# alexlocher/hpmvs

Hardware: AMD Instinct MI355X
Metric: refined_patches_per_sec (higher is better)
Workload: dtype f32 textures / f64 optimiser

## Files before the change

hpmvs_amd/api.py:

```python
from __future__ import annotations

import ctypes as C
import os
from dataclasses import dataclass

import numpy as np

try:
    import torch
except Exception:
    torch = None

HERE = os.path.dirname(os.path.abspath(__file__))
LIB_PATH = os.environ.get("HPMVS_LIB") or os.path.join(HERE, "libhpmvs_amd.so")
MAX_IMAGES = 256
FAST_IMAGES = 64
MAX_LEVELS = 8


class HpmvsError(RuntimeError):
    pass


class Options(C.Structure):
# ... 4 lines not shown

class Camera(C.Structure):
    _fields_ = [("P0", C.c_float * 12), ("center", C.c_float * 4), ("xaxis", C.c_float * 3),
                ("yaxis", C.c_float * 3), ("zaxis", C.c_float * 3), ("fsum", C.c_float), ("n_levels", C.c_int32)]


class PatchBatch(C.Structure):
    _fields_ = [("n", C.c_int32), ("max_images", C.c_int32), ("center", C.c_void_p), ("normal", C.c_void_p),
                ("scale", C.c_void_p), ("n_images", C.c_void_p), ("images", C.c_void_p), ("ok", C.c_void_p),
                ("color", C.c_void_p), ("ncc", C.c_void_p), ("fmin", C.c_void_p), ("x", C.c_void_p),
                ("result", C.c_void_p), ("nevals", C.c_void_p), ("stage", C.c_void_p), ("ngrabs", C.c_void_p)]


class LeafTable(C.Structure):
    _fields_ = [("n", C.c_int32), ("root_center", C.c_float * 3), ("root_width", C.c_float), ("cell_center", C.c_void_p),
                ("cell_width", C.c_void_p), ("patch_center", C.c_void_p), ("born", C.c_void_p), ("died", C.c_void_p)]


class OctreeIndex(C.Structure):
    _fields_ = [("root_center", C.c_float * 3), ("root_width", C.c_float), ("n_branches", C.c_int32), ("n_leaves", C.c_int32),
                ("branch_key", C.c_void_p), ("leaf_key", C.c_void_p)]


class SeedTreeInfo(C.Structure):
    _fields_ = [("root_center", C.c_float * 3), ("root_width", C.c_float), ("scale_floor", C.c_float), ("n_rows", C.c_int32),
                ("n_leaves", C.c_int32)]


EXPORTS = [
    "hpmvs_last_error", "hpmvs_device_count", "hpmvs_build_id", "hpmvs_default_options", "hpmvs_camera_from_nvm",
    "hpmvs_scene_create", "hpmvs_scene_set_view", "hpmvs_scene_set_covis", "hpmvs_scene_commit",
    "hpmvs_scene_destroy", "hpmvs_scene_get_level", "hpmvs_scene_bytes", "hpmvs_build_pyramid",
    "hpmvs_optimize_batch", "hpmvs_init_patches_batch", "hpmvs_objective_batch", "hpmvs_inccs_batch", "hpmvs_last_kernel_ms",
    "hpmvs_last_wide_patches",
    "hpmvs_expand_batch", "hpmvs_expand_directions", "hpmvs_selftest_bobyqa",
    "hpmvs_pack_records", "hpmvs_unpack_records", "hpmvs_allgather_records", "hpmvs_pack_record_tails", "hpmvs_unpack_record_tails",
    "hpmvs_scene_depth_reset", "hpmvs_scene_depth_set_level", "hpmvs_scene_depth_get_level",
    "hpmvs_set_depths_batch", "hpmvs_depth_gates_batch", "hpmvs_depth_footprints_batch", "hpmvs_depth_ops_batch", "hpmvs_level_support_batch",
    "hpmvs_host_alloc", "hpmvs_host_free", "hpmvs_last_staging",
    "hpmvs_undistort", "hpmvs_undistort_map", "hpmvs_scene_set_view_distorted",
    "hpmvs_regularize_batch", "hpmvs_filter_batch", "hpmvs_seed_tree_batch", "hpmvs_octree_locate_batch",
]

_lib = None


def lib():
    global _lib
    if _lib is not None:
        return _lib
    if not os.path.exists(LIB_PATH):
        raise HpmvsError(f"{LIB_PATH} is missing: run `python -c 'import __graft_entry__ as g; g.build()'` "
                         "(there is no fallback implementation)")
    L = C.CDLL(LIB_PATH)
    L.hpmvs_last_error.restype = C.c_char_p
    L.hpmvs_build_id.restype = C.c_char_p
    L.hpmvs_default_options.argtypes = [C.POINTER(Options)]
    L.hpmvs_camera_from_nvm.argtypes = [C.c_double, C.POINTER(C.c_double), C.POINTER(C.c_double), C.c_int, C.c_int,
                                        C.c_int, C.POINTER(Camera)]
    L.hpmvs_scene_create.argtypes = [C.c_int, C.c_int, C.POINTER(C.c_void_p)]
    L.hpmvs_scene_set_view.argtypes = [C.c_void_p, C.c_int, C.c_int, C.c_int, C.c_void_p, C.c_int, C.POINTER(Camera)]
    L.hpmvs_scene_set_covis.argtypes = [C.c_void_p, C.c_int, C.POINTER(C.c_int32), C.c_int]
    L.hpmvs_scene_commit.argtypes = [C.c_void_p]
    L.hpmvs_scene_destroy.argtypes = [C.c_void_p]
    L.hpmvs_scene_get_level.argtypes = [C.c_void_p, C.c_int, C.c_int, C.c_void_p, C.c_size_t, C.POINTER(C.c_int),
                                        C.POINTER(C.c_int)]
    L.hpmvs_scene_bytes.restype = C.c_size_t
# ... 131 lines not shown
        _chk(L.hpmvs_scene_commit(self.h))

    def close(self):
        if self.h:
            lib().hpmvs_scene_destroy(self.h)
            self.h = C.c_void_p()

    def __del__(self):
        try:
            self.close()
        except Exception:
            pass

    def bytes(self) -> int:
        return lib().hpmvs_scene_bytes(self.h)

    def level(self, view: int, level: int) -> np.ndarray:
        w, h = C.c_int(), C.c_int()
        _chk(lib().hpmvs_scene_get_level(self.h, view, level, None, 0, C.byref(w), C.byref(h)))
        out = np.empty((h.value, w.value, 3), dtype=np.uint8)
        _chk(lib().hpmvs_scene_get_level(self.h, view, level, out.ctypes.data, out.nbytes, C.byref(w), C.byref(h)))
        return out

    def last_staging(self):
        a, b = C.c_ulonglong(), C.c_ulonglong()
        _chk(lib().hpmvs_last_staging(self.h, C.byref(a), C.byref(b)))
        return a.value, b.value

    def last_wide_patches(self) -> int:
        n = C.c_int32()
        _chk(lib().hpmvs_last_wide_patches(self.h, C.byref(n)))
        return n.value

    def last_kernel_ms(self) -> float:
        ms = C.c_float()
        _chk(lib().hpmvs_last_kernel_ms(self.h, C.byref(ms)))
        return ms.value


class Batch:

    def __init__(self, center, normal, scale, n_images, images):
        self.n = int(len(scale))
        self.max_images = int(images.shape[1])
        self.center = np.ascontiguousarray(center, dtype=np.float32).copy()
        self.normal = np.ascontiguousarray(normal, dtype=np.float32).copy()
        self.scale = np.ascontiguousarray(scale, dtype=np.float32).copy()
        self.n_images = np.ascontiguousarray(n_images, dtype=np.int32).copy()
        self.images = np.ascontiguousarray(images, dtype=np.int32).copy()
        n = self.n
        self.ok = np.zeros(n, dtype=np.uint8)
        self.color = np.zeros((n, 3), dtype=np.float32)
        self.ncc = np.zeros(n, dtype=np.float32)
        self.fmin = np.zeros(n, dtype=np.float64)
        self.x = np.zeros((n, 3), dtype=np.float64)
        self.result = np.zeros(n, dtype=np.int32)
        self.nevals = np.zeros(n, dtype=np.int32)
        self.stage = np.zeros(n, dtype=np.int32)
        self.ngrabs = np.zeros(n, dtype=np.int32)

    @classmethod
    def from_seeds(cls, seeds, idx=None):
        if idx is None:
            idx = np.arange(len(seeds.scale))
        idx = np.asarray(idx)
        return cls(seeds.center[idx], seeds.normal[idx], seeds.scale[idx], seeds.n_images[idx], seeds.images[idx])
# ... 240 lines not shown
```

hpmvs_amd/csrc/capi.hip:

```cpp
#include <hip/hip_runtime.h>

#include <dlfcn.h>

#include <algorithm>
#include <atomic>
#include <chrono>
#include <cmath>
#include <cstdio>
#include <cstdlib>
#include <cstring>
#include <mutex>
#include <optional>
#include <string>
#include <thread>
#include <time.h>
#include <vector>

#include "../../include/hpmvs_amd.h"
#include "dev_types.h"
#include "launch.h"
#include "octree.hpp"

using namespace hpmvs;

// ... 1726 lines not shown
    HIPCHK(hipGetLastError());
    return c.finish();
}

int hpmvs_depth_footprints_batch(const hpmvs_scene* s, const hpmvs_patch_batch* b, int32_t* writes, int32_t* frees,
                                 int32_t* attached, int32_t* view_block, int on_device, void* stream) {
    int rc = check_depth_batch(s, b, "depth_footprints_batch");
    if (rc) return rc;
    if (!writes && !frees && !attached && !view_block) return fail(HPMVS_ERR_ARG, "depth_footprints_batch: no output array");
    if (b->n == 0) return HPMVS_OK;
    HIPCHK(hipSetDevice(s->device));
    hipStream_t st = (hipStream_t)stream;
    Call c(s, on_device, st);
    const size_t n = (size_t)b->n, M = (size_t)b->max_images, V = (size_t)s->n_views;
    const DevBatch D = c.batch(b, Call::kRead);
    int32_t *dw = c.out(writes, n * M * 4), *df = c.out(frees, n * M * 4);
    int32_t *da = c.out(attached, n * M * 3), *dv = c.out(view_block, n * V * 3);
    if ((rc = c.begin())) return rc;
    launch_depth_footprints(dev_scene(s), s->ddepth, D, dw, df, da, dv, st);
    HIPCHK(hipGetLastError());
    return c.finish();
}

int hpmvs_last_wide_patches(const hpmvs_scene* s, int32_t* n) {
    if (!s || !n) return fail(HPMVS_ERR_ARG, "last_wide_patches: null argument");
    *n = 0;
    if (!s->last_ws) return HPMVS_OK;
    HIPCHK(hipSetDevice(s->device));
    HIPCHK(hipDeviceSynchronize());
    HIPCHK(hipMemcpy(n, s->last_ws + 241, sizeof(int32_t), hipMemcpyDeviceToHost));
    return HPMVS_OK;
}

int hpmvs_debug_counters(const hpmvs_scene* s, unsigned long long* out4) {
    if (!s || !out4) return fail(HPMVS_ERR_ARG, "debug_counters: null argument");
    HIPCHK(hipSetDevice(s->device));
    { const int rcq = service_quiesce(s); if (rcq) return rcq; }
    HIPCHK(hipDeviceSynchronize());
    if (!s->last_queue) return fail(HPMVS_ERR_STATE, "debug_counters: no launch yet");
    HIPCHK(hipMemcpy(out4, (char*)s->last_queue + 16, 544, hipMemcpyDeviceToHost));
    return HPMVS_OK;
}

int hpmvs_last_staging(const hpmvs_scene* s, unsigned long long* staged_bytes, unsigned long long* in_place_bytes) {
    if (!s || !staged_bytes || !in_place_bytes) return fail(HPMVS_ERR_ARG, "last_staging: null argument");
    *staged_bytes = s->last_staged_bytes; *in_place_bytes = s->last_mapped_bytes;
    return HPMVS_OK;
}

void* hpmvs_host_alloc(size_t bytes) {
    void* p = nullptr;
    if (bytes == 0 || hipHostMalloc(&p, bytes, hipHostMallocDefault) != hipSuccess) { (void)hipGetLastError(); return nullptr; }
    return p;
}
void hpmvs_host_free(void* p) {
    if (p && hipHostFree(p) != hipSuccess) (void)hipGetLastError();
}

int hpmvs_last_kernel_ms(const hpmvs_scene* s, float* ms) {
    if (!s || !ms) return fail(HPMVS_ERR_ARG, "last_kernel_ms: null argument");
    if (!s->timed) return fail(HPMVS_ERR_STATE, "last_kernel_ms: no optimize launch yet");
    HIPCHK(hipSetDevice(s->device));
    HIPCHK(hipEventSynchronize(s->ev1));
    HIPCHK(hipEventElapsedTime(ms, s->ev0, s->ev1));
    return HPMVS_OK;
}
// ... 3 lines not shown
```

hpmvs_amd/csrc/kernel_optimize.hip:

```cpp
#include <hip/hip_runtime.h>
#include <atomic>

#include "prof.h"
#define BQ_STATE_LDS 1
#define BQ_STATE_LDS_EXTERN 1
#ifndef BQ_P
#define BQ_P 29
#endif
#define BQ_SLOTS BQ_P
#ifndef HPMVS_STATIC_SLOTS
#define HPMVS_STATIC_SLOTS (!HPMVS_COLD_GLOBAL)
#endif
#ifndef HPMVS_STATIC_MAX_PER_WG
#define HPMVS_STATIC_MAX_PER_WG(W_, kS_) ((W_) * (kS_))
#endif
#ifndef HPMVS_SPREAD_SOLO
#define HPMVS_SPREAD_SOLO 1
#endif
#ifndef HPMVS_COLD_GLOBAL
#define HPMVS_COLD_GLOBAL 0
#endif
#if HPMVS_COLD_GLOBAL
#define BQ_COLD_GLOBAL 1
#ifndef BQ_COLD_LO
#define BQ_COLD_LO 77
#endif
#ifndef BQ_COLD_HI
#define BQ_COLD_HI 138
#endif
#define HPMVS_STATE_ND (164 - (BQ_COLD_HI - BQ_COLD_LO))
#else
#define HPMVS_STATE_ND 164
#endif
#define HPMVS_STATE_NI 13
#define HPMVS_REGION_BYTES (HPMVS_STATE_ND * 8 * BQ_P + HPMVS_STATE_NI * 4 * BQ_P)
#define HPMVS_REGION_KIB ((HPMVS_REGION_BYTES + 1023) / 1024)
#define HPMVS_REGION_16 (HPMVS_REGION_KIB * 64)
#ifndef HPMVS_WG_WAVES
#define HPMVS_WG_WAVES 8
#endif
#ifndef HPMVS_WG_REGIONS
#if HPMVS_COLD_GLOBAL
#define HPMVS_WG_REGIONS 6
#else
#define HPMVS_WG_REGIONS 4
#endif
#endif
#ifdef HPMVS_VARIANT_SUFFIX
#define HPMVS_CAT2(a, b) a##b
#define HPMVS_CAT(a, b) HPMVS_CAT2(a, b)
#define HPMVS_V(name) HPMVS_CAT(name, HPMVS_VARIANT_SUFFIX)
#define HPMVS_VK(name) HPMVS_CAT(name, HPMVS_VARIANT_SUFFIX)
#else
#define HPMVS_VK(name) name
#define HPMVS_V(name) name##_std
#endif
extern __shared__ uint4 hpmvs_dyn[];
#define bq_lds_d ((double*)hpmvs_dyn)
#define bq_lds_i ((int*)((char*)hpmvs_dyn + HPMVS_STATE_ND * 8 * BQ_P))
#include "bobyqa3.hpp"
#include "launch.h"
#include "photometric.hpp"
#include "pipeline.hpp"

namespace hpmvs {

static_assert(BQ_ND_LDS == HPMVS_STATE_ND && BQ_NI == HPMVS_STATE_NI, "state region sized for another layout");

namespace {

constexpr int kP = BQ_P;
constexpr int kRow = 64;
constexpr size_t kCounterBytes = 1024;
constexpr int kPark16 = HPMVS_REGION_16;

#ifndef HPMVS_PARK_AUX
#define HPMVS_PARK_AUX 0
#endif
#ifndef HPMVS_PROXY
#define HPMVS_PROXY 0
#endif
constexpr int kAuxDoubles = 64;
constexpr int kAuxVal = 18;
constexpr int kAuxGrabs = 25;
constexpr int kAuxCtx = 64;
constexpr int kMaxExtra = 7;
typedef __attribute__((address_space(1))) double gdouble;
typedef __attribute__((address_space(1))) float gfloat;
__device__ __forceinline__ void page_in(const uint4* __restrict__ park, uint4* hpmvs_region) {
    const char* g = (const char*)(park + lane_id());
#pragma unroll
    for (int c4 = 0; c4 < HPMVS_REGION_KIB; c4 += 4) {
        asm volatile("" : "+v"(g));
        auto lds = (__attribute__((address_space(3))) void*)(hpmvs_region + c4 * 64);
        auto src = (const __attribute__((address_space(1))) void*)g;
        __builtin_amdgcn_global_load_lds(src, lds, 16, 0, HPMVS_PARK_AUX);
        if (c4 + 1 < HPMVS_REGION_KIB) __builtin_amdgcn_global_load_lds(src, lds, 16, 1024, HPMVS_PARK_AUX);
        if (c4 + 2 < HPMVS_REGION_KIB) __builtin_amdgcn_global_load_lds(src, lds, 16, 2048, HPMVS_PARK_AUX);
        if (c4 + 3 < HPMVS_REGION_KIB) __builtin_amdgcn_global_load_lds(src, lds, 16, 3072, HPMVS_PARK_AUX);
        g += 4096;
    }
    asm volatile("s_waitcnt vmcnt(0)" ::: "memory");
}
#ifndef HPMVS_PARK_NT_STORE
#define HPMVS_PARK_NT_STORE 0
#endif
#if HPMVS_PARK_NT_STORE
#define HPMVS_PARK_ST(dst, v) __builtin_nontemporal_store((v), &(dst))
#else
#define HPMVS_PARK_ST(dst, v) (dst) = (v)
#endif
__device__ __attribute__((noinline)) void page_out(uint4* __restrict__ park, int region_index) {
    typedef unsigned int u4 __attribute__((ext_vector_type(4)));
    typedef __attribute__((address_space(1))) u4 gu4;
    const int lane = lane_id();
    const u4* region = (const u4*)(hpmvs_dyn + region_index * HPMVS_REGION_16);
    gu4* out = (gu4*)(unsigned long long)park;
    int c = 0;
#pragma unroll
    for (; c + 8 <= HPMVS_REGION_KIB; c += 8) {
        const u4 v0 = region[(c + 0) * 64 + lane], v1 = region[(c + 1) * 64 + lane], v2 = region[(c + 2) * 64 + lane],
                    v3 = region[(c + 3) * 64 + lane], v4 = region[(c + 4) * 64 + lane], v5 = region[(c + 5) * 64 + lane],
                    v6 = region[(c + 6) * 64 + lane], v7 = region[(c + 7) * 64 + lane];
        __builtin_amdgcn_sched_barrier(0);
        HPMVS_PARK_ST(out[(c + 0) * 64 + lane], v0); HPMVS_PARK_ST(out[(c + 1) * 64 + lane], v1); HPMVS_PARK_ST(out[(c + 2) * 64 + lane], v2); HPMVS_PARK_ST(out[(c + 3) * 64 + lane], v3);
        HPMVS_PARK_ST(out[(c + 4) * 64 + lane], v4); HPMVS_PARK_ST(out[(c + 5) * 64 + lane], v5); HPMVS_PARK_ST(out[(c + 6) * 64 + lane], v6); HPMVS_PARK_ST(out[(c + 7) * 64 + lane], v7);
        __builtin_amdgcn_sched_barrier(0);
    }
#pragma unroll
    for (; c < HPMVS_REGION_KIB; c++) { const u4 v = region[c * 64 + lane]; HPMVS_PARK_ST(out[c * 64 + lane], v); }
}

}

__device__ __forceinline__ unsigned long long ld_host64(const unsigned long long* p) {
    return __hip_atomic_load(p, __ATOMIC_RELAXED, __HIP_MEMORY_SCOPE_SYSTEM);
}

#ifndef HPMVS_WAVES_PER_EU
#define HPMVS_WAVES_PER_EU 2
#endif
#ifndef HPMVS_BQ_PRIO
#define HPMVS_BQ_PRIO 3
#endif
#ifndef HPMVS_LOCK_SLEEP
#define HPMVS_LOCK_SLEEP 8
#endif
#ifndef HPMVS_A_PRIO
#define HPMVS_A_PRIO 2
#endif
template <bool SERVICE, int W, int R>
__device__ __forceinline__ void optimize_body(DevScene sc, DevOptions o, DevBatch b, int32_t* queue) {
    const int lane = lane_id();
    const int wv = (int)(threadIdx.x >> 6);
    int* const hpmvs_lock = (int*)(hpmvs_dyn + R * HPMVS_REGION_16);
    const int n_wgs = (int)gridDim.x;
    const int gw = wv * n_wgs + (int)blockIdx.x;
    uint16_t* lists = (uint16_t*)((char*)queue + kCounterBytes) + (size_t)gw * kP * kRow;
    uint16_t* row = &lists[(lane < kP ? lane : 0) * kRow];
    uint4* park = (uint4*)((char*)queue + kCounterBytes + (size_t)W * n_wgs * kP * kRow * sizeof(uint16_t)) + (size_t)gw * kPark16;
#if HPMVS_COLD_GLOBAL
    char* cold = (char*)queue + kCounterBytes + (size_t)W * n_wgs * kP * kRow * sizeof(uint16_t) + (size_t)W * n_wgs * kPark16 * 16 +
                 (size_t)W * n_wgs * kP * kRow * sizeof(float) + (size_t)gw * BQ_NCOLD * kP * sizeof(double);
    {
// ... 17 lines not shown
    int px_k = 0;

    constexpr bool service = SERVICE;
    const int per_wg = (b.n + n_wgs - 1) / n_wgs;
    int quota = per_wg - wv * kP;
    quota = quota < 0 ? 0 : (quota < kP ? quota : kP);
#if HPMVS_SPREAD_SOLO
    if (4 * per_wg <= 3 * R * kP) {
        const int a = per_wg < R ? per_wg : R;
        quota = wv < a ? per_wg / a + (wv < per_wg % a ? 1 : 0) : 0;
    }
#endif
#if HPMVS_STATIC_SLOTS
    constexpr bool can_static = !SERVICE && (W % R == 0) && (W / R > 1);
    constexpr int kS = kP / (W / R > 0 ? W / R : 1);
    bool stat = false;
    if (can_static && per_wg <= HPMVS_STATIC_MAX_PER_WG(W, kS)) {
        stat = true;
        const int a = per_wg < W ? per_wg : W;
        quota = wv < a ? per_wg / a + (wv < per_wg % a ? 1 : 0) : 0;
    }
#endif
    if (service) quota = wv == 0 ? (b.svc_lanes < kP ? b.svc_lanes : kP) : 0;
    if (threadIdx.x <= R) hpmvs_lock[threadIdx.x] = 0;
    __syncthreads();
    if (quota == 0) {
        if (lane == 0) atomicOr(&hpmvs_lock[R], 1 << wv);
        return;
    }
    __builtin_amdgcn_s_setprio(HPMVS_A_PRIO);
    bool held = false, solo = false;
    int reg = 0;
    bool parked = false;
    int stage = (lane < quota) ? S_FETCH : S_IDLE;
    int idx = -1, nimg = 0, ii = 0, refindex = -1, ngrabs = 0, fail_stage = 0, nl_result = 0;
    float c0[3] = {0, 0, 0}, n0[3] = {0, 0, 0};
    float c[3] = {0, 0, 0}, n[3] = {0, 0, 1};
    float scale = 1.0f, refbest = 0.0f;
    OptFields F;
    Bobyqa3 B;
    B.slot = lane < kP ? lane : 0;
    B.slot_i = B.slot;
#if HPMVS_STATIC_SLOTS
    if (stat) {
        reg = wv / (W / R);
        const int sl = (lane < kS ? lane : 0) + (wv % (W / R)) * kS;
        B.slot = sl + reg * (HPMVS_REGION_16 * 2);
        B.slot_i = sl + reg * (HPMVS_REGION_16 * 4);
        held = true; solo = true;
    }
#endif
#if HPMVS_COLD_GLOBAL
    B.coff = (unsigned)B.slot * 8u;
    B.coldp = cold;
    B.cold = __builtin_amdgcn_make_buffer_rsrc(cold, 0, BQ_NCOLD * BQ_CSTRIDE * 8, 0x00020000);
#endif
    float ax[3] = {0, 0, 0}, ay[3] = {0, 0, 0}, az[3] = {0, 0, 1};
    int op = OP_NONE, req_ref = 0, req_robust = 0;
    float req_thr = 0.0f;
    double res_f = 0.0;
    unsigned long long res_mask = 0ull;
    float res_sum = 0.0f;
    const double lbv[3] = {-HUGE_VAL, -23.99999, -23.99999};
    const double ubv[3] = {HUGE_VAL, 23.99999, 23.99999};

#ifdef HPMVS_PROFILE_PHASES
    long long tA = 0, tB = 0, nrounds = 0, nreq = 0, t0 = clock64();
    s_prof[lane] = 0ull;
    __syncthreads();
#endif
    int res_n = 0, res_fail = 0;
    float res_rgb[3] = {0, 0, 0};
    int svc_n = 0, svc_closed = 0;
    uint32_t* srec = service ? b.svc_stage + ((size_t)gw * kP + (lane < kP ? lane : 0)) * kSvcOutDwords : nullptr;
    int fin_idx = 0;
    bool fin_pending = false;
    for (;;) {
        bool yield = false;
        if (service) {
            if (gw == 0 && lane == 0) {
                const int closed = __hip_atomic_load(&b.svc_ctrl[1], __ATOMIC_RELAXED, __HIP_MEMORY_SCOPE_SYSTEM);
                asm volatile("s_waitcnt vmcnt(0)" ::: "memory");
                const int n_pub = __hip_atomic_load(&b.svc_ctrl[0], __ATOMIC_RELAXED, __HIP_MEMORY_SCOPE_SYSTEM);
                __hip_atomic_store(&queue[200], n_pub, __ATOMIC_RELAXED, __HIP_MEMORY_SCOPE_AGENT);
                asm volatile("s_waitcnt vmcnt(0)" ::: "memory");
                __hip_atomic_store(&queue[201], closed, __ATOMIC_RELAXED, __HIP_MEMORY_SCOPE_AGENT);
            }
            int cl = 0, np = 0;
            if (lane == 0) {
                cl = __hip_atomic_load(&queue[201], __ATOMIC_RELAXED, __HIP_MEMORY_SCOPE_AGENT);
                asm volatile("s_waitcnt vmcnt(0)" ::: "memory");
                np = __hip_atomic_load(&queue[200], __ATOMIC_RELAXED, __HIP_MEMORY_SCOPE_AGENT);
            }
            svc_closed = bcast_i(cl, 0);
            svc_n = bcast_i(np, 0);
        }
        while (op == OP_NONE && stage != S_IDLE && !yield) {
            bool finish_fail = false, finish_ok = false;
            switch (stage) {
            case S_FETCH:
                idx = atomicAdd(queue, 1);
// ... 133 lines not shown
                break;
            }
            default: stage = S_IDLE; break;
            }
            if (finish_ok || finish_fail) {
                if (service) {
                    srec[0] = finish_ok ? 1u : 0u; srec[1] = (unsigned)(finish_ok ? 0 : fail_stage); srec[2] = (unsigned)nl_result;
                    srec[4] = (unsigned)ngrabs; srec[5] = (unsigned)(finish_ok ? nimg : 0);
                    if (finish_ok) {
                        for (int k = 0; k < 3; k++) { srec[8 + k] = __float_as_uint(c[k]); srec[12 + k] = __float_as_uint(n[k]); srec[16 + k] = __float_as_uint(res_rgb[k]); }
                        srec[11] = __float_as_uint(1.0f); srec[15] = __float_as_uint(0.0f);
                        srec[19] = __float_as_uint(1.4f);
                        for (int k = 0; k < nimg && k < b.max_images; k++) srec[32 + k] = row[k];
                    }
                    fin_idx = idx; fin_pending = true; yield = true;
                } else {
                    b.ok[idx] = finish_ok ? 1 : (fail_stage == 100 ? 2 : 0);
                    if (finish_ok) {
                        for (int k = 0; k < 3; k++) { b.center[4 * idx + k] = c[k]; b.normal[4 * idx + k] = n[k]; }
                        b.center[4 * idx + 3] = 1.0f;
                        b.normal[4 * idx + 3] = 0.0f;
                        b.n_images[idx] = nimg;
                        for (int k = 0; k < nimg && k < b.max_images; k++) b.images[(size_t)idx * b.max_images + k] = row[k];
                        if (b.color) { b.color[3 * idx] = res_rgb[0]; b.color[3 * idx + 1] = res_rgb[1]; b.color[3 * idx + 2] = res_rgb[2]; }
                        if (b.ncc) b.ncc[idx] = 1.4f;
                    }
                    if (b.stage) b.stage[idx] = finish_ok ? 0 : fail_stage;
                    if (b.result) b.result[idx] = nl_result;
                    if (b.ngrabs) b.ngrabs[idx] = ngrabs;
                }
                stage = S_FETCH;
            }
        }
        if (service) {
            const unsigned long long fm = __ballot(fin_pending);
            if (fm) {
                asm volatile("s_waitcnt vmcnt(0)" ::: "memory");
                for (unsigned long long t = fm; t; t &= t - 1ull) {
                    const int p = __ffsll((long long)t) - 1;
                    const int pidx = bcast_i(fin_idx, p);
                    const uint32_t* src = b.svc_stage + ((size_t)gw * kP + p) * kSvcOutDwords;
                    uint32_t* dst = b.svc_out + (size_t)pidx * kSvcOutDwords;
                    const uint32_t v0 = __hip_atomic_load(src + lane, __ATOMIC_RELAXED, __HIP_MEMORY_SCOPE_AGENT);
                    const uint32_t v1 = lane < kSvcOutDwords - 64 ? __hip_atomic_load(src + 64 + lane, __ATOMIC_RELAXED, __HIP_MEMORY_SCOPE_AGENT) : 0u;
                    __hip_atomic_store(dst + lane, v0, __ATOMIC_RELAXED, __HIP_MEMORY_SCOPE_SYSTEM);
                    if (lane < kSvcOutDwords - 64) __hip_atomic_store(dst + 64 + lane, v1, __ATOMIC_RELAXED, __HIP_MEMORY_SCOPE_SYSTEM);
                }
                asm volatile("s_waitcnt vmcnt(0)" ::: "memory");
                if (fin_pending) __hip_atomic_store(&b.svc_done[fin_idx], 1, __ATOMIC_RELAXED, __HIP_MEMORY_SCOPE_SYSTEM);
                fin_pending = false;
            }
        }
        {
            wave_lds_sync();
            const unsigned long long lm = __ballot(op >= OPL_ADD && op <= OPL_F3);
            if (lm) {
                BQ_PROF_BEGIN(tls_);
                for (unsigned long long t = lm; t; t &= t - 1ull) {
                    const int p = __ffsll((long long)t) - 1;
                    const int kind = bcast_i(op, p);
                    uint16_t* prow = lists + p * kRow;
                    const int pn = bcast_i(nimg, p);
                    const U3 pc{bcast_f(c[0], p), bcast_f(c[1], p), bcast_f(c[2], p)};
                    const U3 pnrm{bcast_f(n[0], p), bcast_f(n[1], p), bcast_f(n[2], p)};
                    const float pscale = bcast_f(scale, p);
                    const unsigned long long pmask = bcast_u64(res_mask, p);
                    ListResult r;
                    r.nimg = 0; r.fail = 0; r.rgb = U3{0.0f, 0.0f, 0.0f};
                    const ListEnv le = list_env(sc, o);
                    if (kind == OPL_ADD) r.nimg = coop_add_images(le, prow, pn, pc, pnrm, pscale);
                    else if (kind == OPL_F1) r = coop_list_f1(le, prow, pn, pmask, pc, pnrm, pscale);
                    else if (kind == OPL_F2) r = coop_list_f2(le, prow, pn, pmask, pc, pnrm);
                    else { LevelThr lt; for (int k = 0; k < kMaxLevels; k++) lt.t[k] = sc.lvl_thr[k]; r = coop_list_f3(sc.views, lt, o.MIN_IMAGES_PER_PATCH, prow, pn, pmask, pc, pscale, b.max_images, service || b.color != nullptr); }
                    if (lane == p) {
                        res_n = r.nimg; res_fail = r.fail;
                        res_rgb[0] = r.rgb.x; res_rgb[1] = r.rgb.y; res_rgb[2] = r.rgb.z;
                        op = OP_NONE;
                    }
                }
                wave_lds_sync();
                BQ_PROF_END(tls_, 24);
                continue;
            }
        }
        if (__any(op >= OPQ_START)) {
            const bool mine = op >= OPQ_START;
            double x0[3] = {0, 0, 0}, dx[3] = {1, 1, 1};
            if (op == OPQ_START) {
                parameters_from_center_norm(F, o, n, lbv, ubv, x0);
                bq_default_step(x0, lbv, ubv, dx);
            }
            if (!held) {
                BQ_PROF_BEGIN(tpg_);
                int got = 0;
                if (lane == 0) {
                    int r = R > 1 ? wv % R : 0;
                    for (;;) {
                        if (atomicCAS(&hpmvs_lock[r], 0, 1 + wv) == 0) break;
                        r = r + 1 == R ? 0 : r + 1;
                        if (r == (R > 1 ? wv % R : 0)) __builtin_amdgcn_s_sleep(HPMVS_LOCK_SLEEP);
                    }
                    got = r;
                }
                reg = __builtin_amdgcn_readfirstlane(got);
                __builtin_amdgcn_fence(__ATOMIC_ACQUIRE, "workgroup");
                __builtin_amdgcn_wave_barrier();
                BQ_PROF_END(tpg_, 25);
                B.slot = (lane < kP ? lane : 0) + reg * (HPMVS_REGION_16 * 2);
                B.slot_i = (lane < kP ? lane : 0) + reg * (HPMVS_REGION_16 * 4);
                BQ_PROF_BEGIN(tpi_);
                if (parked) page_in(park, hpmvs_dyn + reg * HPMVS_REGION_16);
                BQ_PROF_END(tpi_, 27);
                held = true;
                solo = W - __popc((unsigned)hpmvs_lock[R] & ((1u << W) - 1u)) <= R;
            }
#if HPMVS_BQ_PRIO
            __builtin_amdgcn_s_setprio(HPMVS_BQ_PRIO);
#endif
            int ret = BQ_DONE;
#ifdef HPMVS_HOLD_DELAY
            for (int dly = 0; dly < HPMVS_HOLD_DELAY; dly++) __builtin_amdgcn_s_sleep(127);
#endif
            if (kProxy) {
                if (op == OPQ_START) {
                    ret = bq_start(B, x0, lbv, ubv, dx, 1.e-7, 1000, (double*)(unsigned long long)aux);
                    pre_nf = ret == BQ_CONTINUE ? 1 : 0; pre_ctx = false;
                }
                const bool pre = op == OPQ_STEP && pre_nf > 0;
                bool stepping = op == OPQ_STEP;
                double fcur = res_f;
                int kx = 0;
                for (;;) {
                    if (stepping) { ret = bq_step(B, fcur); pre_nf += pre ? 1 : 0; }
                    stepping = pre && kx < extra && ret == BQ_CONTINUE;
                    if (!__any(stepping)) break;
                    if (stepping) { fcur = (double)aux[kAuxVal + kx]; ngrabs += (int)aux[kAuxGrabs + kx]; kx++; }
                }
                if (pre) { if (pre_nf > 7 || ret != BQ_CONTINUE) pre_nf = 0; extra = 0; }
            } else {
                if (op == OPQ_START) ret = bq_start(B, x0, lbv, ubv, dx, 1.e-7, 1000);
                if (op == OPQ_STEP) ret = bq_step(B, res_f);
            }
            double xe[3] = {0, 0, 0};
            if (mine) {
                for (int k = 0; k < 3; k++) xe[k] = BQA(xeval, k);
                if (ret != BQ_CONTINUE) {
                    nl_result = BQN(rc);
                    if (service) {
                        const unsigned long long mf = (unsigned long long)__double_as_longlong((double)BQS(minf));
                        srec[3] = (unsigned)BQN(nevals);
                        srec[20] = (unsigned)mf; srec[21] = (unsigned)(mf >> 32);
                        for (int k = 0; k < 3; k++) {
                            const unsigned long long xv = (unsigned long long)__double_as_longlong(xe[k]);
                            srec[22 + 2 * k] = (unsigned)xv; srec[23 + 2 * k] = (unsigned)(xv >> 32);
                        }
                    } else {
                        if (b.fmin) b.fmin[idx] = BQS(minf);
                        if (b.x) for (int k = 0; k < 3; k++) b.x[3 * idx + k] = xe[k];
                        if (b.nevals) b.nevals[idx] = BQN(nevals);
                    }
                }
            }
            if (!solo) {
                BQ_PROF_BEGIN(tpo_);
                page_out(park, reg);
                parked = true;
                __builtin_amdgcn_fence(__ATOMIC_RELEASE, "workgroup");
                __builtin_amdgcn_wave_barrier();
                if (lane == 0) atomicExch(&hpmvs_lock[reg], 0);
                held = false;
                BQ_PROF_END(tpo_, 26);
            }
#if HPMVS_BQ_PRIO
            __builtin_amdgcn_s_setprio(HPMVS_A_PRIO);
#endif
            {
                const bool cont = mine && ret == BQ_CONTINUE;
                const bool failed = mine && !cont && (op == OPQ_START || !(nl_result >= 1 && nl_result <= 4));
                const bool done = mine && !cont && !failed;
                int nset = (cont || done) ? 1 : 0;
                const int pfirst = pre_nf;
                if (kProxy) {
                    const bool anyfree = __any(!mine && op == OP_NONE && lane < kP && (stage == S_IDLE || (service && stage == S_WAIT)));
                    if (anyfree && cont && pre_nf >= 1 && pre_nf <= 6 && !pre_ctx) { nset = 8 - pre_nf; pre_ctx = true; }
                }
                for (int k = 0; __any(k < nset); k++) {
                    if (k < nset) {
                        double xk[3] = {xe[0], xe[1], xe[2]};
                        float ck[3], nk[3];
                        if (kProxy && k > 0) for (int i3 = 0; i3 < 3; i3++) xk[i3] = aux[3 * (pfirst + k - 2) + i3];
                        set_center_norm(F, o, xk, ck, nk);
                        if (k == 0) { for (int i3 = 0; i3 < 3; i3++) { c[i3] = ck[i3]; n[i3] = nk[i3]; } }
                        else if (kProxy) {
                            gfloat* ctx = (gfloat*)aux + kAuxCtx + 8 + 6 * (pfirst + k - 2);
                            for (int i3 = 0; i3 < 3; i3++) { ctx[i3] = ck[i3]; ctx[3 + i3] = nk[i3]; }
                            gfloat* c0 = (gfloat*)aux + kAuxCtx;
                            c0[0] = scale; c0[1] = __int_as_float(nimg);
                        }
                    }
                }
                if (cont) op = OP_OBJ;
                else if (failed) { op = OP_NONE; stage = S_BQFAIL; }
                else if (done) { op = OPL_ADD; stage = S_ADD2; }
            }
// ... 9 lines not shown
            unsigned long long own = freem ? __ballot(want > 0) : 0ull;
            if (own) {
                for (; own && freem; own &= own - 1ull) {
                    const int p = __ffsll((long long)own) - 1;
                    const int w = bcast_i(want, p);
                    int cnt = 0;
                    for (; cnt < w && freem; cnt++, freem &= freem - 1ull)
                        if (lane == __ffsll((long long)freem) - 1) { px_owner = p; px_k = cnt; }
                    if (lane == p) extra = cnt;
                }
                const int src = px_owner >= 0 ? px_owner : lane;
                const int o_op = shfl_i(op, src), o_ref = shfl_i(req_ref, src), o_pre = shfl_i(pre_nf, src);
                if (px_owner >= 0) {
                    brow = lists + px_owner * kRow;
                    const gfloat* ctx = (const gfloat*)(auxw + px_owner * kAuxDoubles) + kAuxCtx;
                    scale = ctx[0]; nimg = __float_as_int(ctx[1]);
                    const gfloat* cn = (o_op == OP_OBJ) ? ctx + 8 + 6 * (o_pre - 1 + px_k) : ctx + 2;
                    for (int k = 0; k < 3; k++) { c[k] = cn[k]; n[k] = cn[3 + k]; }
                    if (o_op == OP_OBJ) op = OP_OBJ;
                    else { op = OP_REFSUM; req_ref = o_ref + 1 + px_k; req_robust = 1; }
                }
            }
        }
        BQ_PROF_BEGIN(tax_);
        if (op != OP_NONE) {
            const DevView& RV = sc.views[brow[op == OP_OBJ ? 0 : req_ref]];
            calc_patch_axes(RV.xaxis, RV.yaxis, n, scale, ax, ay, az);
        }
        BQ_PROF_END(tax_, 17);
        wave_lds_sync();
        unsigned long long pending = __ballot(op != OP_NONE);
#ifdef HPMVS_PROFILE_PHASES
        { const long long t1 = clock64(); tA += t1 - t0; t0 = t1; nrounds++; nreq += __popcll(pending); }
#endif
        if (pending == 0ull) {
            if (service && (__any(stage != S_IDLE) || (gw == 0 && !svc_closed))) {
                if (gw == 0) __builtin_amdgcn_s_sleep(32);
                else { __builtin_amdgcn_s_sleep(127); __builtin_amdgcn_s_sleep(127); __builtin_amdgcn_s_sleep(127); }
                continue;
            }
            if (lane == 0) atomicOr(&hpmvs_lock[R], 1 << wv);
            break;
        }
        {
            PackedReq q;
            q.obj_mode = (op == OP_OBJ) ? 1 : 0;
            q.ref = req_ref; q.robust = req_robust; q.nimg = nimg; q.thr = req_thr;
            q.scale = scale;
            for (int k = 0; k < 3; k++) { q.c[k] = c[k]; q.zax[k] = (op == OP_OBJ) ? az[k] : n[k]; q.px[k] = ax[k]; q.py[k] = ay[k]; }
            PackedRes r;
            r.obj = 2.0; r.keep = 0ull; r.incc_sum = 0.0f; r.ngrabs = 0;
            __builtin_amdgcn_s_setprio(0);
            wave_eval_rows<false>(sc, o, brow, pending, q, r, erows);
            __builtin_amdgcn_s_setprio(HPMVS_A_PRIO);
            if (op != OP_NONE) {
                res_f = r.obj;
                res_mask = r.keep;
                res_sum = r.incc_sum;
                ngrabs += r.ngrabs;
                op = OP_NONE;
            }
            if (kProxy) {
                const unsigned long long pm = __ballot(px_owner >= 0);
                if (pm) {
                    for (unsigned long long t = pm; t; t &= t - 1ull) {
                        const int fl = __ffsll((long long)t) - 1;
                        const int p = bcast_i(px_owner, fl), k = bcast_i(px_k, fl), g = bcast_i(r.ngrabs, fl), kind = bcast_i(q.obj_mode, fl);
                        const double vf = bcast_d(res_f, fl);
                        const float vs = bcast_f(res_sum, fl);
                        if (lane == p) { aux[kAuxVal + k] = kind ? vf : (double)vs; aux[kAuxGrabs + k] = (double)g; }
                    }
                    asm volatile("s_waitcnt vmcnt(0)" ::: "memory");
                    px_owner = -1;
                }
            }
        }
        wave_lds_sync();
#ifdef HPMVS_PROFILE_PHASES
        { const long long t1 = clock64(); tB += t1 - t0; t0 = t1; }
#endif
    }
#ifdef HPMVS_PROFILE_PHASES
    unsigned long long* dbg = (unsigned long long*)(queue + 4);
    if (lane == 0) {
        atomicAdd(&dbg[0], (unsigned long long)tA);
        atomicAdd(&dbg[1], (unsigned long long)tB);
        atomicAdd(&dbg[2], (unsigned long long)nrounds);
        atomicAdd(&dbg[3], (unsigned long long)nreq);
    }
    __syncthreads();
    if (threadIdx.x == 0)
        for (int k = 0; k < 64; k++) atomicAdd(&dbg[4 + k], s_prof[k]);
#endif
}

__global__ void __launch_bounds__(64 * HPMVS_WG_WAVES, HPMVS_WAVES_PER_EU) HPMVS_VK(optimize_kernel)(DevScene sc, DevOptions o, DevBatch b, int32_t* queue) {
    optimize_body<false, HPMVS_WG_WAVES, HPMVS_WG_REGIONS>(sc, o, b, queue);
}
#ifndef HPMVS_VARIANT_SUFFIX
__global__ void __launch_bounds__(128, HPMVS_WAVES_PER_EU) optimize_service_kernel(DevScene sc, DevOptions o, DevBatch b, int32_t* queue) {
    optimize_body<true, 2, 1>(sc, o, b, queue);
}
#endif

static size_t lds_bytes(int regions) { return (size_t)regions * HPMVS_REGION_16 * 16 + (size_t)(regions + 1) * sizeof(int); }

static int max_workgroups(int n_cus, int waves, int regions) {
    int lds_per_wg = (int)lds_bytes(regions);
#ifdef HPMVS_PROFILE_PHASES
    lds_per_wg += 64 * 8;
#endif
    lds_per_wg = (lds_per_wg + 511) & ~511;
    int per_cu = (160 * 1024) / lds_per_wg;
    if (per_cu > 4 * HPMVS_WAVES_PER_EU / waves) per_cu = 4 * HPMVS_WAVES_PER_EU / waves;
    return n_cus * per_cu;
}

size_t HPMVS_V(optimize_workspace_bytes)(int n_cus) {
    const size_t waves = (size_t)HPMVS_WG_WAVES * max_workgroups(n_cus, HPMVS_WG_WAVES, HPMVS_WG_REGIONS);
    return kCounterBytes + waves * kP * kRow * sizeof(uint16_t) + waves * (size_t)kPark16 * 16 + waves * kP * kRow * sizeof(float) +
           waves * (size_t)(HPMVS_COLD_GLOBAL ? (164 - HPMVS_STATE_ND) : 0) * kP * sizeof(double) +
           (HPMVS_PROXY == 2 ? waves * kP * kAuxDoubles * sizeof(double) : 0);
}

#ifndef HPMVS_VARIANT_SUFFIX
size_t optimize_workspace_bytes_for(int wgs) {
    return kCounterBytes + (size_t)2 * wgs * kP * kRow * sizeof(uint16_t) + (size_t)2 * wgs * (size_t)kPark16 * 16 +
           (size_t)2 * wgs * kP * kRow * sizeof(float) + (size_t)2 * wgs * (size_t)(HPMVS_COLD_GLOBAL ? (164 - HPMVS_STATE_ND) : 0) * kP * sizeof(double) +
           (HPMVS_PROXY ? (size_t)2 * wgs * kP * kAuxDoubles * sizeof(double) : 0);
}
size_t optimize_stage_bytes_for(int wgs) { return (size_t)2 * wgs * kP * kSvcOutDwords * sizeof(uint32_t); }
void launch_optimize_service(const DevScene& sc, const DevOptions& o, const DevBatch& b, int32_t* workspace, int wgs,
                             hipStream_t st) {
    hipLaunchKernelGGL(optimize_service_kernel, dim3(wgs), dim3(128), lds_bytes(1), st, sc, o, b, workspace);
}
#endif

void HPMVS_V(launch_optimize)(const DevScene& sc, const DevOptions& o, const DevBatch& b, int32_t* workspace, int n_cus,
                     hipStream_t st) {
    if (b.n <= 0) return;
    int wgs = b.n;
    const int cap = max_workgroups(n_cus, HPMVS_WG_WAVES, HPMVS_WG_REGIONS);
    if (wgs > cap) wgs = cap;
// ... 11 lines not shown
```

hpmvs_amd/csrc/kernel_optimize_big.hip:

```cpp
#ifndef HPMVS_BIG_P
#define HPMVS_BIG_P 64
#endif
#define BQ_P HPMVS_BIG_P
#ifndef BQ_COLD_HI
#define BQ_COLD_HI 145
#endif
#ifndef HPMVS_COLD_GLOBAL
#define HPMVS_COLD_GLOBAL 1
#endif
#ifndef HPMVS_WG_REGIONS
#define HPMVS_WG_REGIONS 3
#endif
#ifndef HPMVS_SPLIT_PREP
#define HPMVS_SPLIT_PREP 0
#endif
#ifndef HPMVS_SINGLE_FAST
#define HPMVS_SINGLE_FAST 1
#endif
#ifndef HPMVS_PARK_AUX
#define HPMVS_PARK_AUX 2
#endif
#ifndef HPMVS_PARK_NT_STORE
#define HPMVS_PARK_NT_STORE 1
#endif
#define HPMVS_VARIANT_SUFFIX _big
#include "kernel_optimize.hip"
```

hpmvs_amd/csrc/kernel_optimize_big_tree.hip:

```cpp
#ifndef HPMVS_BIG_P
#define HPMVS_BIG_P 64
#endif
#define BQ_P HPMVS_BIG_P
#ifndef BQ_COLD_HI
#define BQ_COLD_HI 145
#endif
#ifndef HPMVS_COLD_GLOBAL
#define HPMVS_COLD_GLOBAL 1
#endif
#ifndef HPMVS_WG_REGIONS
#define HPMVS_WG_REGIONS 3
#endif
#define HPMVS_FAST_SUMS 1
#ifndef HPMVS_SPLIT_PREP
#define HPMVS_SPLIT_PREP 0
#endif
#ifndef HPMVS_SINGLE_FAST
#define HPMVS_SINGLE_FAST 0
#endif
#ifndef HPMVS_PARK_AUX
#define HPMVS_PARK_AUX 2
#endif
#ifndef HPMVS_PARK_NT_STORE
#define HPMVS_PARK_NT_STORE 1
#endif
#define HPMVS_VARIANT_SUFFIX _big_tree
#include "kernel_optimize.hip"
```

hpmvs_amd/csrc/prof.h:

```cpp
#pragma once
#if defined(HPMVS_PROFILE_PHASES) && defined(__HIPCC__)
#include <hip/hip_runtime.h>
static __device__ unsigned long long g_bqprof[64];
static __shared__ unsigned long long s_prof[64];
#endif
```

include/hpmvs_amd.h:

```cpp
#ifndef HPMVS_AMD_H
#define HPMVS_AMD_H

#include <stddef.h>
#include <stdint.h>

#ifdef __cplusplus
extern "C" {
#endif

#define HPMVS_OK 0
#define HPMVS_ERR_HIP (-1)
#define HPMVS_ERR_ARG (-2)
#define HPMVS_ERR_STATE (-3)
#define HPMVS_ERR_NODEVICE (-4)

#define HPMVS_MAX_LEVELS 8
#define HPMVS_MAX_IMAGES 256
#define HPMVS_FAST_IMAGES 64
#define HPMVS_RECORD_IMAGES 64

typedef struct hpmvs_scene hpmvs_scene;

typedef struct {
    int32_t MAXLEVEL;
// ... 112 lines not shown
                       int32_t *keep, int on_device, void *stream);

typedef struct {
    float root_center[3];
    float root_width;
    float scale_floor;
    int32_t n_rows;
    int32_t n_leaves;
} hpmvs_seed_tree_info;
int hpmvs_seed_tree_batch(hpmvs_scene *s, hpmvs_patch_batch *b, int patch_init_maxlevel, int set_depths,
                          hpmvs_seed_tree_info *info, int32_t *rows , int32_t *cell_start ,
                          float *cell_center , float *cell_width , int32_t *cell_level ,
                          float *patch_center , int on_device, void *stream);

typedef struct {
    float root_center[3];
    float root_width;
    int32_t n_branches;
    int32_t n_leaves;
    const uint64_t *branch_key;
    const uint64_t *leaf_key;
} hpmvs_octree_index;
int hpmvs_octree_locate_batch(const hpmvs_scene *s, const hpmvs_octree_index *t, int n, const float *points ,
                              const float *add_width , uint8_t *inside , uint64_t *leaf_key ,
                              int32_t *leaf_index , float *leaf_width , float *leaf_center ,
                              uint64_t *target_key , int on_device, void *stream);

void *hpmvs_host_alloc(size_t bytes);
void hpmvs_host_free(void *p);
int hpmvs_last_staging(const hpmvs_scene *s, unsigned long long *staged_bytes, unsigned long long *in_place_bytes);

int hpmvs_last_kernel_ms(const hpmvs_scene *s, float *ms);
int hpmvs_last_wide_patches(const hpmvs_scene *s, int32_t *n);

typedef struct hpmvs_record {
    float center[4];
    float normal[4];
    float color[3];
    float scale;
    double fmin;
    uint8_t ok;
    uint8_t pad0;
    uint16_t n_images;
    uint8_t pad1[4];
    uint16_t images[HPMVS_RECORD_IMAGES];
} hpmvs_record;
typedef struct hpmvs_record_tail {
    int32_t patch;
    uint16_t count;
    uint16_t pad;
    uint16_t images[HPMVS_MAX_IMAGES - HPMVS_RECORD_IMAGES];
} hpmvs_record_tail;
int hpmvs_pack_record_tails(const hpmvs_patch_batch *b, hpmvs_record_tail *tails, int32_t cap, int32_t *n_tails, void *stream);
int hpmvs_unpack_record_tails(const hpmvs_record_tail *tails, int32_t n_tails, int32_t patch_offset, hpmvs_patch_batch *b, void *stream);
int hpmvs_pack_records(const hpmvs_patch_batch *b, hpmvs_record *records, void *stream);
int hpmvs_unpack_records(const hpmvs_record *records, int n, hpmvs_patch_batch *b, void *stream);
int hpmvs_allgather_records(void *nccl_comm, const hpmvs_record *send, size_t count, hpmvs_record *recv, void *stream);

int hpmvs_selftest_bobyqa(int device, int n, const int32_t *kind, const double *params, const double *x0,
                          const double *lb, const double *ub, int maxeval, double *xfinal, double *minf,
                          int32_t *result, int32_t *nevals, int32_t *rescue_calls, double *trace, int trace_cap);

#ifdef __cplusplus
}
#endif
#endif
// ... 1 lines not shown
```

Baseline: 5.201 million.

## Let tail waves share an LDS region via resident windows during ramp-down

Adds a resident ramp-down mode to the big and big_tree optimiser variants. Once the work queue is drained and a wave has few live lanes, the wave flags itself ready. When every wave in the workgroup is flagged, up to three waves can hold a slot window inside one LDS region and keep their BOBYQA state there, instead of locking the whole region and paging state in and out on every round. It also adds profiling counters for the drain phase and an API call that reports how many waves went resident. The gain is meant to be less lock contention and paging traffic in the tail, at the cost of more complex lock-word logic and a risk of slot collisions or deadlock.

Result: no change. 5.230 million (median of 6 runs) (+0.6%).

```diff
diff --git a/hpmvs_amd/api.py b/hpmvs_amd/api.py
--- a/hpmvs_amd/api.py
+++ b/hpmvs_amd/api.py
@@ -60,7 +60,7 @@
     "hpmvs_scene_create", "hpmvs_scene_set_view", "hpmvs_scene_set_covis", "hpmvs_scene_commit",
     "hpmvs_scene_destroy", "hpmvs_scene_get_level", "hpmvs_scene_bytes", "hpmvs_build_pyramid",
     "hpmvs_optimize_batch", "hpmvs_init_patches_batch", "hpmvs_objective_batch", "hpmvs_inccs_batch", "hpmvs_last_kernel_ms",
-    "hpmvs_last_wide_patches",
+    "hpmvs_last_wide_patches", "hpmvs_last_resident_waves",
     "hpmvs_expand_batch", "hpmvs_expand_directions", "hpmvs_selftest_bobyqa",
     "hpmvs_pack_records", "hpmvs_unpack_records", "hpmvs_allgather_records", "hpmvs_pack_record_tails", "hpmvs_unpack_record_tails",
     "hpmvs_scene_depth_reset", "hpmvs_scene_depth_set_level", "hpmvs_scene_depth_get_level",
@@ -258,6 +258,11 @@
         _chk(lib().hpmvs_last_wide_patches(self.h, C.byref(n)))
         return n.value
 
+    def last_resident_waves(self) -> int:
+        n = C.c_int32()
+        _chk(lib().hpmvs_last_resident_waves(self.h, C.byref(n)))
+        return n.value
+
     def last_kernel_ms(self) -> float:
         ms = C.c_float()
         _chk(lib().hpmvs_last_kernel_ms(self.h, C.byref(ms)))
diff --git a/hpmvs_amd/csrc/capi.hip b/hpmvs_amd/csrc/capi.hip
--- a/hpmvs_amd/csrc/capi.hip
+++ b/hpmvs_amd/csrc/capi.hip
@@ -1782,6 +1782,26 @@
     return HPMVS_OK;
 }
 
+int hpmvs_last_resident_waves(const hpmvs_scene* s, int32_t* n) {
+    if (!s || !n) return fail(HPMVS_ERR_ARG, "last_resident_waves: null argument");
+    *n = 0;
+    if (!s->last_ws) return HPMVS_OK;
+    HIPCHK(hipSetDevice(s->device));
+    HIPCHK(hipDeviceSynchronize());
+    HIPCHK(hipMemcpy(n, s->last_ws + 210, sizeof(int32_t), hipMemcpyDeviceToHost));
+    return HPMVS_OK;
+}
+
+int hpmvs_debug_counters_drain(const hpmvs_scene* s, unsigned long long* out16) {
+    if (!s || !out16) return fail(HPMVS_ERR_ARG, "debug_counters_drain: null argument");
+    HIPCHK(hipSetDevice(s->device));
+    { const int rcq = service_quiesce(s); if (rcq) return rcq; }
+    HIPCHK(hipDeviceSynchronize());
+    if (!s->last_queue) return fail(HPMVS_ERR_STATE, "debug_counters_drain: no launch yet");
+    HIPCHK(hipMemcpy(out16, (char*)s->last_queue + 16 + 544, 128, hipMemcpyDeviceToHost));
+    return HPMVS_OK;
+}
+
 int hpmvs_debug_counters(const hpmvs_scene* s, unsigned long long* out4) {
     if (!s || !out4) return fail(HPMVS_ERR_ARG, "debug_counters: null argument");
     HIPCHK(hipSetDevice(s->device));
diff --git a/hpmvs_amd/csrc/kernel_optimize.hip b/hpmvs_amd/csrc/kernel_optimize.hip
--- a/hpmvs_amd/csrc/kernel_optimize.hip
+++ b/hpmvs_amd/csrc/kernel_optimize.hip
@@ -45,6 +45,9 @@
 #else
 #define HPMVS_WG_REGIONS 4
 #endif
+#endif
+#ifndef HPMVS_RESIDENT_RAMPDOWN
+#define HPMVS_RESIDENT_RAMPDOWN 0
 #endif
 #ifdef HPMVS_VARIANT_SUFFIX
 #define HPMVS_CAT2(a, b) a##b
@@ -73,6 +76,7 @@
 constexpr int kRow = 64;
 constexpr size_t kCounterBytes = 1024;
 constexpr int kPark16 = HPMVS_REGION_16;
+constexpr int kResidentWord = 210;
 
 #ifndef HPMVS_PARK_AUX
 #define HPMVS_PARK_AUX 0
@@ -130,6 +134,21 @@
 #pragma unroll
     for (; c < HPMVS_REGION_KIB; c++) { const u4 v = region[c * 64 + lane]; HPMVS_PARK_ST(out[c * 64 + lane], v); }
 }
+#if HPMVS_RESIDENT_RAMPDOWN
+constexpr int kWinPerRegion = 3;
+constexpr int kWinSlots = kP / kWinPerRegion;
+__device__ __attribute__((noinline)) void gather_window(const uint4* __restrict__ park, int slot_d, int slot_i, bool live) {
+    if (!live) return;
+    const int lane = lane_id();
+    const gdouble* pd = (const gdouble*)(unsigned long long)park + lane;
+    const __attribute__((address_space(1))) int* pi =
+        (const __attribute__((address_space(1))) int*)(unsigned long long)((const char*)park + HPMVS_STATE_ND * 8 * kP) + lane;
+#pragma unroll 8
+    for (int i = 0; i < HPMVS_STATE_ND; i++) bq_lds_d[i * kP + slot_d] = pd[i * kP];
+#pragma unroll
+    for (int i = 0; i < HPMVS_STATE_NI; i++) bq_lds_i[i * kP + slot_i] = pi[i * kP];
+}
+#endif
 
 }
 
@@ -213,6 +232,14 @@
     bool held = false, solo = false;
     int reg = 0;
     bool parked = false;
+#if HPMVS_RESIDENT_RAMPDOWN
+    constexpr bool kResident = !SERVICE && W <= 8 && R <= 8 && R * kWinPerRegion >= W && kWinSlots >= 1;
+    bool rdy = false;
+#endif
+#ifdef HPMVS_PROFILE_PHASES
+    bool drained = false;
+    long long tdrain = 0;
+#endif
     int stage = (lane < quota) ? S_FETCH : S_IDLE;
     int idx = -1, nimg = 0, ii = 0, refindex = -1, ngrabs = 0, fail_stage = 0, nl_result = 0;
     float c0[3] = {0, 0, 0}, n0[3] = {0, 0, 0};
@@ -248,6 +275,7 @@
 #ifdef HPMVS_PROFILE_PHASES
     long long tA = 0, tB = 0, nrounds = 0, nreq = 0, t0 = clock64();
     s_prof[lane] = 0ull;
+    if (lane < 16) s_prof[64 + lane] = 0ull;
     __syncthreads();
 #endif
     int res_n = 0, res_fail = 0;
@@ -447,6 +475,17 @@
                 stage = S_FETCH;
             }
         }
+#if defined(HPMVS_PROFILE_PHASES) || HPMVS_RESIDENT_RAMPDOWN
+#endif
+#ifdef HPMVS_PROFILE_PHASES
+        if (!service && !drained && __any(stage == S_IDLE && idx >= b.n)) { drained = true; tdrain = clock64(); }
+#endif
+#if HPMVS_RESIDENT_RAMPDOWN
+        if (kResident && !rdy && __any(stage == S_IDLE && idx >= b.n) && __popcll(__ballot(stage != S_IDLE)) <= kWinSlots) {
+            if (lane == 0) atomicOr(&hpmvs_lock[R], 0x100 << wv);
+            rdy = true;
+        }
+#endif
         if (service) {
             const unsigned long long fm = __ballot(fin_pending);
             if (fm) {
@@ -508,6 +547,31 @@
             if (!held) {
                 BQ_PROF_BEGIN(tpg_);
                 int got = 0;
+#if HPMVS_RESIDENT_RAMPDOWN
+                if (lane == 0) {
+                    int r = R > 1 ? wv % R : 0;
+                    for (;;) {
+                        if (atomicCAS(&hpmvs_lock[r], 0, 1 + wv) == 0) {
+                            if (!kResident) break;
+                            __builtin_amdgcn_fence(__ATOMIC_ACQUIRE, "workgroup");
+                            const unsigned word = (unsigned)__hip_atomic_load(&hpmvs_lock[R], __ATOMIC_RELAXED, __HIP_MEMORY_SCOPE_WORKGROUP);
+                            if (((word | (word >> 8)) & ((1u << W) - 1u)) != (1u << W) - 1u) break;
+                            const int taken = (int)((word >> (16 + 2 * r)) & 3u);
+                            if (taken < kWinPerRegion) {
+                                atomicAdd(&hpmvs_lock[R], 1 << (16 + 2 * r));
+                                got = (1 + taken) << 8;
+                                break;
+                            }
+                            atomicExch(&hpmvs_lock[r], 0);
+                        }
+                        r = r + 1 == R ? 0 : r + 1;
+                        if (r == (R > 1 ? wv % R : 0)) __builtin_amdgcn_s_sleep(HPMVS_LOCK_SLEEP);
+                    }
+                    got |= r;
+                }
+                got = __builtin_amdgcn_readfirstlane(got);
+                reg = got & 0xff;
+#else
                 if (lane == 0) {
                     int r = R > 1 ? wv % R : 0;
                     for (;;) {
@@ -518,17 +582,40 @@
                     got = r;
                 }
                 reg = __builtin_amdgcn_readfirstlane(got);
+#endif
                 __builtin_amdgcn_fence(__ATOMIC_ACQUIRE, "workgroup");
                 __builtin_amdgcn_wave_barrier();
-                BQ_PROF_END(tpg_, 25);
+                BQ_PROF_END(tpg_, (drained ? 32 : 25));
+#if HPMVS_RESIDENT_RAMPDOWN
+                if (kResident && (got >> 8)) {
+                    const unsigned long long livem = __ballot(stage != S_IDLE);
+                    const int sl = ((got >> 8) - 1) * kWinSlots + (stage != S_IDLE ? __popcll(livem & ((1ull << lane) - 1ull)) : 0);
+                    B.slot = sl + reg * (HPMVS_REGION_16 * 2);
+                    B.slot_i = sl + reg * (HPMVS_REGION_16 * 4);
+                    if (parked) gather_window(park, B.slot, B.slot_i, stage != S_IDLE);
+                    parked = false;
+                    __builtin_amdgcn_fence(__ATOMIC_RELEASE, "workgroup");
+                    __builtin_amdgcn_wave_barrier();
+                    if (lane == 0) { atomicExch(&hpmvs_lock[reg], 0); atomicAdd(&queue[kResidentWord], 1); }
+                    held = true; solo = true;
+                } else
+#endif
+                {
                 B.slot = (lane < kP ? lane : 0) + reg * (HPMVS_REGION_16 * 2);
                 B.slot_i = (lane < kP ? lane : 0) + reg * (HPMVS_REGION_16 * 4);
                 BQ_PROF_BEGIN(tpi_);
                 if (parked) page_in(park, hpmvs_dyn + reg * HPMVS_REGION_16);
-                BQ_PROF_END(tpi_, 27);
+                BQ_PROF_END(tpi_, (drained ? 33 : 27));
                 held = true;
                 solo = W - __popc((unsigned)hpmvs_lock[R] & ((1u << W) - 1u)) <= R;
-            }
+                }
+            }
+#ifdef HPMVS_PROFILE_PHASES
+            if (drained) {
+                const unsigned long long nlive = (unsigned long long)__popcll(__ballot(stage != S_IDLE));
+                if (lane == 0) { atomicAdd(&s_prof[70], 1ull); atomicAdd(&s_prof[71], nlive); atomicAdd(&s_prof[72], solo ? 1ull : 0ull); }
+            }
+#endif
 #if HPMVS_BQ_PRIO
             __builtin_amdgcn_s_setprio(HPMVS_BQ_PRIO);
 #endif
@@ -584,7 +671,7 @@
                 __builtin_amdgcn_wave_barrier();
                 if (lane == 0) atomicExch(&hpmvs_lock[reg], 0);
                 held = false;
-                BQ_PROF_END(tpo_, 26);
+                BQ_PROF_END(tpo_, (drained ? 34 : 26));
             }
 #if HPMVS_BQ_PRIO
             __builtin_amdgcn_s_setprio(HPMVS_A_PRIO);
@@ -660,6 +747,10 @@
         unsigned long long pending = __ballot(op != OP_NONE);
 #ifdef HPMVS_PROFILE_PHASES
         { const long long t1 = clock64(); tA += t1 - t0; t0 = t1; nrounds++; nreq += __popcll(pending); }
+        if (drained) {
+            const unsigned long long nlive = (unsigned long long)__popcll(__ballot(stage != S_IDLE));
+            if (lane == 0) { atomicAdd(&s_prof[73], 1ull); atomicAdd(&s_prof[74], nlive); }
+        }
 #endif
         if (pending == 0ull) {
             if (service && (__any(stage != S_IDLE) || (gw == 0 && !svc_closed))) {
@@ -715,10 +806,11 @@
         atomicAdd(&dbg[1], (unsigned long long)tB);
         atomicAdd(&dbg[2], (unsigned long long)nrounds);
         atomicAdd(&dbg[3], (unsigned long long)nreq);
+        if (drained) { atomicAdd(&s_prof[75], (unsigned long long)(clock64() - tdrain)); atomicAdd(&s_prof[76], 1ull); }
     }
     __syncthreads();
     if (threadIdx.x == 0)
-        for (int k = 0; k < 64; k++) atomicAdd(&dbg[4 + k], s_prof[k]);
+        for (int k = 0; k < 80; k++) atomicAdd(&dbg[4 + k], s_prof[k]);
 #endif
 }
 
@@ -736,7 +828,7 @@
 static int max_workgroups(int n_cus, int waves, int regions) {
     int lds_per_wg = (int)lds_bytes(regions);
 #ifdef HPMVS_PROFILE_PHASES
-    lds_per_wg += 64 * 8;
+    lds_per_wg += 80 * 8;
 #endif
     lds_per_wg = (lds_per_wg + 511) & ~511;
     int per_cu = (160 * 1024) / lds_per_wg;
diff --git a/hpmvs_amd/csrc/kernel_optimize_big.hip b/hpmvs_amd/csrc/kernel_optimize_big.hip
--- a/hpmvs_amd/csrc/kernel_optimize_big.hip
+++ b/hpmvs_amd/csrc/kernel_optimize_big.hip
@@ -23,5 +23,8 @@
 #ifndef HPMVS_PARK_NT_STORE
 #define HPMVS_PARK_NT_STORE 1
 #endif
+#ifndef HPMVS_RESIDENT_RAMPDOWN
+#define HPMVS_RESIDENT_RAMPDOWN 1
+#endif
 #define HPMVS_VARIANT_SUFFIX _big
 #include "kernel_optimize.hip"
diff --git a/hpmvs_amd/csrc/kernel_optimize_big_tree.hip b/hpmvs_amd/csrc/kernel_optimize_big_tree.hip
--- a/hpmvs_amd/csrc/kernel_optimize_big_tree.hip
+++ b/hpmvs_amd/csrc/kernel_optimize_big_tree.hip
@@ -24,5 +24,8 @@
 #ifndef HPMVS_PARK_NT_STORE
 #define HPMVS_PARK_NT_STORE 1
 #endif
+#ifndef HPMVS_RESIDENT_RAMPDOWN
+#define HPMVS_RESIDENT_RAMPDOWN 1
+#endif
 #define HPMVS_VARIANT_SUFFIX _big_tree
 #include "kernel_optimize.hip"
diff --git a/hpmvs_amd/csrc/prof.h b/hpmvs_amd/csrc/prof.h
--- a/hpmvs_amd/csrc/prof.h
+++ b/hpmvs_amd/csrc/prof.h
@@ -2,5 +2,5 @@
 #if defined(HPMVS_PROFILE_PHASES) && defined(__HIPCC__)
 #include <hip/hip_runtime.h>
 static __device__ unsigned long long g_bqprof[64];
-static __shared__ unsigned long long s_prof[64];
+static __shared__ unsigned long long s_prof[80];
 #endif
diff --git a/include/hpmvs_amd.h b/include/hpmvs_amd.h
--- a/include/hpmvs_amd.h
+++ b/include/hpmvs_amd.h
@@ -168,6 +168,7 @@
 
 int hpmvs_last_kernel_ms(const hpmvs_scene *s, float *ms);
 int hpmvs_last_wide_patches(const hpmvs_scene *s, int32_t *n);
+int hpmvs_last_resident_waves(const hpmvs_scene *s, int32_t *n);
 
 typedef struct hpmvs_record {
     float center[4];
```
